# shubhamchandak94/HARC

Hardware: AMD Instinct MI355X
Metric: Mreads/s reorder+encode, 100 bp (higher is better)
Workload: dtype u64 (2-bit packed bases, XOR+popcount)

## Files before the change

harc_amd/csrc/api.cpp:

```cpp
#include "internal.h"
#include <stdarg.h>
#include <chrono>
#include <stdlib.h>

static thread_local char g_err[512] = "";
void harc_set_error(const char *fmt, ...)
{
    va_list ap; va_start(ap, fmt); vsnprintf(g_err, sizeof g_err, fmt, ap); va_end(ap);
}
extern "C" const char *harc_amd_last_error(void) { return g_err; }

static size_t pool_hand_back(harc_amd_ctx *c, size_t from, size_t asked)
{
    size_t given = 0;
    for (size_t i = 0; i < c->pool.size(); i++) {
        harc_amd_ctx::PoolChunk &k = c->pool[i];
        if (i == from || k.size == 0 || k.used != 0) continue;
        (void)hipFree(k.base); c->pool_total -= k.size; given += k.size; k.base = nullptr; k.size = 0;
    }
    if (given) {
        (void)hipGetLastError();
        if (getenv("HARC_AMD_TRACE")) fprintf(stderr, "[pool] %.2f GB of empty chunks handed back for a request of %.2f GB\n", given / 1e9, asked / 1e9);
    }
    return given;
// ... 166 lines not shown
}

extern "C" void harc_amd_destroy(harc_amd_ctx *c)
{
    if (!c) return;
    (void)hipSetDevice(c->P.device);
    if (c->stream) { (void)hipStreamSynchronize(c->stream); }
    if (c->copy_stream) { (void)hipStreamSynchronize(c->copy_stream); }
    delete c->comm; c->comm = nullptr;
    for (void *p : c->owned) (void)hipFree(p);
    for (auto &k : c->pool) (void)hipFree(k.base);
    for (auto &k : c->harena) (void)hipHostFree(k.base);
    if (c->feed_ring) (void)hipHostFree(c->feed_ring);
    if (c->stream) (void)hipStreamDestroy(c->stream);
    if (c->copy_stream) (void)hipStreamDestroy(c->copy_stream);
    if (c->ev_copy) (void)hipEventDestroy(c->ev_copy);
    delete c;
}

void harc_drop_results(harc_amd_ctx *c)
{
    harc_pool_release(c, 0);
    c->d_order = nullptr; c->d_flag = c->d_pos = c->d_rc = nullptr; c->d_order_s = nullptr; c->d_oreads = nullptr; c->d_sreads = nullptr;
    c->have_s1 = c->have_s2 = c->s1_from_files = false; c->M = c->S = 0;
    c->d_s2_order = c->d_s2_orderN = nullptr; c->n_s2_order = c->n_s2_orderN = 0;
    for (auto it = c->out.begin(); it != c->out.end();) { if (it->first.first < HARC_AMD_IN_ORDER_N) it = c->out.erase(it); else ++it; }
    harc_host_reset(c);
}

int harc_in_reserve(harc_amd_ctx *c, harc_amd_ctx::InBuf *b, size_t bytes)
{
    if (b->p && b->cap >= bytes) return HARC_AMD_OK;
    if (b->p) { harc_raw_free(c, b->p); b->p = nullptr; b->cap = 0; }
    RC_TRY(harc_raw_alloc(c, &b->p, bytes));
    b->cap = bytes;
    return HARC_AMD_OK;
}
void harc_reset_shard(harc_amd_ctx *c)
{
    c->d_reads = (uint64_t *)c->own_reads.p; c->N = c->N_own;
    c->d_nreads3 = (uint64_t *)c->own_nreads3.p; c->NN = c->NN_own;
    c->d_gid = c->d_ngid = nullptr;
    c->replicated = false;
    memset(c->shard_info, 0, sizeof c->shard_info);
    c->C.n_clean = c->N; c->C.n_N = c->NN;
}

// ... 73 lines not shown
    HIP_TRY(hipSetDevice(c->P.device));
    harc_drop_results(c);
    const int L = c->P.readlen;
    c->M = M; c->S = S;
    RC_TRY(dalloc(c, &c->d_order, (size_t)M + 1)); RC_TRY(dalloc(c, &c->d_flag, (size_t)M + 1)); RC_TRY(dalloc(c, &c->d_pos, (size_t)M + 1));
    RC_TRY(dalloc(c, &c->d_rc, (size_t)M + 1)); RC_TRY(dalloc(c, &c->d_order_s, (size_t)S + 1));
    RC_TRY(dalloc(c, &c->d_oreads, (size_t)M * c->W + 1)); RC_TRY(dalloc(c, &c->d_sreads, (size_t)S * c->W + 1));
    if (M) {
        HIP_TRY(hipMemcpyAsync(c->d_order, order, (size_t)M * 4, hipMemcpyHostToDevice, c->stream));
        HIP_TRY(hipMemcpyAsync(c->d_flag, flag, M, hipMemcpyHostToDevice, c->stream));
        HIP_TRY(hipMemcpyAsync(c->d_pos, pos, M, hipMemcpyHostToDevice, c->stream));
        HIP_TRY(hipMemcpyAsync(c->d_rc, rc, M, hipMemcpyHostToDevice, c->stream));
        char *d = nullptr; RC_TRY(upload(c, temp_dna, (size_t)(M - 1) * (L + 1) + L, &d));
        RC_TRY(s1_pack_ascii(c, d, M, (uint32_t)L + 1, c->d_oreads));
        HIP_TRY(hipStreamSynchronize(c->stream)); harc_raw_free(c, d);
    }
    if (S) {
        HIP_TRY(hipMemcpyAsync(c->d_order_s, order_s, (size_t)S * 4, hipMemcpyHostToDevice, c->stream));
        char *d = nullptr; RC_TRY(upload(c, temp_dna_s, (size_t)(S - 1) * (L + 1) + L, &d));
        RC_TRY(s1_pack_ascii(c, d, S, (uint32_t)L + 1, c->d_sreads));
        HIP_TRY(hipStreamSynchronize(c->stream)); harc_raw_free(c, d);
    }
    HIP_TRY(hipStreamSynchronize(c->stream));
    c->have_s1 = true; c->s1_from_files = true;
    c->C.n_main = M; c->C.n_singleton = S;
    return HARC_AMD_OK;
}

extern "C" int harc_amd_pack_reads_device(harc_amd_ctx *c, const char *d_ascii, uint32_t n, uint32_t stride, uint64_t *d_out)
{
    if (!c || (n && (!d_ascii || !d_out)) || stride < (uint32_t)c->P.readlen) return HARC_AMD_EINVAL;
    HIP_TRY(hipSetDevice(c->P.device));
    RC_TRY(s1_pack_ascii(c, d_ascii, n, stride, d_out));
    HIP_TRY(hipStreamSynchronize(c->stream));
    return HARC_AMD_OK;
}
extern "C" int harc_amd_partition_reads_device(harc_amd_ctx *c, const uint64_t *d_packed, uint32_t n, uint32_t nb, uint64_t *d_out, uint64_t *d_counts)
{
    if (!c || nb == 0 || nb > 4096 || !d_counts || (n && (!d_packed || !d_out))) return HARC_AMD_EINVAL;
    HIP_TRY(hipSetDevice(c->P.device));
    return s1_partition_reads(c, d_packed, n, nb, d_out, reinterpret_cast<unsigned long long *>(d_counts));
}
extern "C" int harc_amd_bucket_reads_device(harc_amd_ctx *c, const uint64_t *d_packed, uint32_t n, uint32_t nb, uint32_t *d_out)
{
    if (!c || nb == 0 || (n && (!d_packed || !d_out))) return HARC_AMD_EINVAL;
    HIP_TRY(hipSetDevice(c->P.device));
    RC_TRY(s1_bucket_reads(c, d_packed, n, nb, d_out));
// ... 18 lines not shown

extern "C" int harc_amd_encode(harc_amd_ctx *c)
{
    if (!c) return HARC_AMD_EINVAL;
    if (!c->have_s1) { harc_set_error("harc_amd_encode: no stage-I result (call harc_amd_reorder or harc_amd_set_stage1_streams)"); return HARC_AMD_ESTATE; }
    HIP_TRY(hipSetDevice(c->P.device));
    const double t0 = now_ms();
    c->s2_part = false; c->s2_e0 = 0; c->s2_e1 = 0;
    uint32_t oi0 = 0, oi1 = 0xFFFFFFFFu;
    int simr = 0, simw = 0;
#ifdef HARC_AMD_EXPERIMENTS
    if (const char *e = getenv("HARC_AMD_S2_SIM")) { if (sscanf(e, "%d/%d", &simr, &simw) != 2 || simw < 2 || simr < 0 || simr >= simw) simw = 0; }
#endif
    const int s2p = getenv("HARC_AMD_S2_PART") ? atoi(getenv("HARC_AMD_S2_PART")) : 1;
    const bool real_part = c->replicated && c->comm && (c->comm->world > 1 || s2p == 2) && s2p != 0;
    if ((real_part || simw) && !c->s1_from_files) {
        const uint32_t E = (uint32_t)c->P.num_thr, wd = real_part ? (uint32_t)c->comm->world : (uint32_t)simw, rk = real_part ? (uint32_t)c->comm->rank : (uint32_t)simr;
        c->s2_world = (int)wd; c->s2_rank = (int)rk;
        c->s2_part = true; c->s2_e0 = (int)((uint64_t)E * rk / wd); c->s2_e1 = (int)((uint64_t)E * (rk + 1) / wd);
        uint32_t q = 1u + (uint32_t)((c->M - 1u) / E); if (q == 0) q = 1;
        const uint64_t a0 = (uint64_t)c->s2_e0 * q, a1 = (uint64_t)c->s2_e1 * q;
        oi0 = (uint32_t)(a0 > c->M ? c->M : a0); oi1 = (uint32_t)((uint32_t)c->s2_e1 >= E || a1 > c->M ? c->M : a1);
    }
    if (!c->s1_from_files) RC_TRY(stage1_make_oriented(c, oi0, oi1));
    RC_TRY(stage2_run(c));
    c->C.encode_ms = now_ms() - t0;
    c->C.total_ms += c->C.encode_ms;
    c->C.device_bytes_peak = c->dev_peak;
    c->have_s2 = true;
    return HARC_AMD_OK;
}

extern "C" int harc_amd_pack_order(harc_amd_ctx *c)
{
    if (!c) return HARC_AMD_EINVAL;
    if (!c->have_s2) { harc_set_error("harc_amd_pack_order: encode first"); return HARC_AMD_ESTATE; }
    HIP_TRY(hipSetDevice(c->P.device));
    return pack_order_run(c);
}

extern "C" int harc_amd_get_stream(harc_amd_ctx *c, int32_t id, int32_t shard, const void **ptr, size_t *len)
{
    if (!c || !ptr || !len) return HARC_AMD_EINVAL;
    *ptr = nullptr; *len = 0;
    HIP_TRY(hipSetDevice(c->P.device));
    auto key = std::make_pair((int)id, (int)shard);
    auto it = c->out.find(key);
    if (it == c->out.end()) {
        if (id >= HARC_AMD_S1_ORDER && id <= HARC_AMD_S1_DNA_SINGLETON) {
            if (!c->have_s1 || shard != 0) { harc_set_error("stream %d not available", id); return HARC_AMD_ESTATE; }
            std::vector<uint8_t> &b = out_buf(c, id, shard);
            const int L = c->P.readlen;
            bool made_oriented = false;
            switch (id) {
            case HARC_AMD_S1_ORDER: RC_TRY(harc_d2h(c, b, c->d_order, (size_t)c->M * 4)); break;
            case HARC_AMD_S1_FLAG: RC_TRY(harc_d2h(c, b, c->d_flag, c->M)); break;
            case HARC_AMD_S1_POS: RC_TRY(harc_d2h(c, b, c->d_pos, c->M)); break;
            case HARC_AMD_S1_RC: RC_TRY(harc_d2h(c, b, c->d_rc, c->M)); break;
            case HARC_AMD_S1_ORDER_SINGLETON: RC_TRY(harc_d2h(c, b, c->d_order_s, (size_t)c->S * 4)); break;
            case HARC_AMD_S1_DNA: {
                if (!c->d_oreads) { RC_TRY(stage1_make_oriented(c)); made_oriented = true; }
                const harc_mark_t mk = harc_pool_mark(c);
                char *d = nullptr; RC_TRY(dalloc(c, &d, (size_t)c->M * (L + 1) + 1));
                RC_TRY(s1_unpack_to_ascii(c, c->d_oreads, c->M, d));
                RC_TRY(harc_d2h(c, b, d, (size_t)c->M * (L + 1)));
                HIP_TRY(hipStreamSynchronize(c->stream)); harc_pool_release(c, mk); (void)made_oriented;
                break; }
            case HARC_AMD_S1_DNA_SINGLETON: {
                const harc_mark_t mk = harc_pool_mark(c);
                uint64_t *sr = c->d_sreads; bool tmp = false;
                if (!sr) { RC_TRY(dalloc(c, &sr, (size_t)c->S * c->W + 1)); tmp = true; RC_TRY(s1_orient(c, c->d_reads, c->d_order_s, nullptr, c->S, sr)); }
                char *d = nullptr; RC_TRY(dalloc(c, &d, (size_t)c->S * (L + 1) + 1));
                RC_TRY(s1_unpack_to_ascii(c, sr, c->S, d));
                RC_TRY(harc_d2h(c, b, d, (size_t)c->S * (L + 1)));
                HIP_TRY(hipStreamSynchronize(c->stream)); harc_pool_release(c, mk); (void)tmp;
                break; }
            }
            HIP_TRY(hipStreamSynchronize(c->stream));
            it = c->out.find(key);
        } else if ((id == HARC_AMD_S2_ORDER || id == HARC_AMD_S2_ORDER_N_PE) && shard == 0 && c->have_s2 && c->d_s2_order) {
            const uint32_t *d = id == HARC_AMD_S2_ORDER ? c->d_s2_order : c->d_s2_orderN;
            const size_t n = id == HARC_AMD_S2_ORDER ? c->n_s2_order : c->n_s2_orderN;
            uint8_t *hp = nullptr;
            RC_TRY(harc_host_alloc(c, (void **)&hp, n));
// ... 43 lines not shown
```

harc_amd/csrc/devutil.h:

```cpp
#pragma once
#include "internal.h"

#define HARC_GRID_ROW 16777215u
static inline dim3 harc_grid256(uint64_t n)
{
    uint64_t b = (n + 255) / 256;
    if (b == 0) b = 1;
    if (b <= HARC_GRID_ROW) return dim3((unsigned)b);
    return dim3(HARC_GRID_ROW, (unsigned)((b + HARC_GRID_ROW - 1) / HARC_GRID_ROW));
}
static inline dim3 harc_fold256(uint64_t nblocks)
{
    if (nblocks == 0) nblocks = 1;
    if (nblocks <= HARC_GRID_ROW) return dim3((unsigned)nblocks);
    return dim3(HARC_GRID_ROW, (unsigned)((nblocks + HARC_GRID_ROW - 1) / HARC_GRID_ROW));
}
static inline dim3 wave_grid(uint32_t n) { if (n <= (1u << 25)) return dim3(n ? n : 1u); return dim3(1u << 25, (n + (1u << 25) - 1) >> 25); }
__device__ __forceinline__ uint64_t harc_bid() { return (uint64_t)blockIdx.y * gridDim.x + blockIdx.x; }
__device__ __forceinline__ uint64_t harc_gid() { return ((uint64_t)blockIdx.y * gridDim.x + blockIdx.x) * blockDim.x + threadIdx.x; }
__device__ __forceinline__ uint32_t harc_gid32()
{
    if (gridDim.y == 1) return blockIdx.x * blockDim.x + threadIdx.x;
    const uint64_t g = harc_gid(); return g > 0xFFFFFFFEull ? 0xFFFFFFFFu : (uint32_t)g;
}
// ... 98 lines not shown
{
    const int r = nb - 64 * w;
    return r >= 64 ? ~(uint64_t)0 : (r <= 0 ? 0 : (((uint64_t)1 << r) - 1));
}
__device__ __forceinline__ uint64_t rev2(uint64_t x)
{
    x = __brevll(x);
    return ((x & 0xAAAAAAAAAAAAAAAAULL) >> 1) | ((x & 0x5555555555555555ULL) << 1);
}
template <int W> __device__ __forceinline__ void rc_words(const uint64_t (&a)[W], int L, uint64_t (&o)[W])
{
    uint64_t r[W];
#pragma unroll
    for (int w = 0; w < W; w++) r[w] = rev2(a[W - 1 - w]);
    const int s = 64 * W - 2 * L;
    const int ws = s >> 6, bs = s & 63;
#pragma unroll
    for (int w = 0; w < W; w++) {
        uint64_t lo = sel0<W>(r, w + ws), hi = sel0<W>(r, w + ws + 1);
        uint64_t v = bs ? ((lo >> bs) | (hi << (64 - bs))) : lo;
        o[w] = (~v) & lowmask_word(2 * L, w);
    }
}
__device__ __forceinline__ uint64_t spread32(uint64_t a)
{
    a &= 0xFFFFFFFFULL;
    a = (a | (a << 16)) & 0x0000FFFF0000FFFFULL;
    a = (a | (a << 8)) & 0x00FF00FF00FF00FFULL;
    a = (a | (a << 4)) & 0x0F0F0F0F0F0F0F0FULL;
    a = (a | (a << 2)) & 0x3333333333333333ULL;
    a = (a | (a << 1)) & 0x5555555555555555ULL;
    return a;
}
__device__ __forceinline__ uint32_t wave_sum_u32(uint32_t v)
{
#pragma unroll
    for (int o = 32; o > 0; o >>= 1) v += __shfl_xor(v, o, 64);
    return v;
}
__device__ __forceinline__ uint64_t shfl_u64(uint64_t x, int src)
{
    const uint32_t lo = __shfl((uint32_t)x, src, 64), hi = __shfl((uint32_t)(x >> 32), src, 64);
    return (uint64_t)lo | ((uint64_t)hi << 32);
}
__device__ __forceinline__ uint64_t shfl_u64_any(uint64_t x, int xormask)
{
// ... 42 lines not shown
```

harc_amd/csrc/internal.h:

```cpp
#pragma once
#include <hip/hip_runtime.h>
#include <stdint.h>
#include <stdio.h>
#include <string.h>
#include <map>
#include <string>
#include <utility>
#include <vector>
#include "../../include/harc_amd.h"

#define HARC_NONE 0xFFFFFFFFu
#define HARC_MAXW 8
#define HARC_MAXW3 12
#define HARC_MAXK (1u << 20)
#define HARC_LOOK_CHUNKS 16
#ifndef HARC_NSUGG
#define HARC_NSUGG 8
#endif

void harc_set_error(const char *fmt, ...);

#define HIP_TRY(expr)                                                                                          \
    do {                                                                                                       \
        hipError_t _e = (expr);                                                                                \
// ... 64 lines not shown
    std::vector<void *> owned;
    std::map<void *, size_t> sizes;
    struct PoolChunk { char *base; size_t size, used; };
    std::vector<PoolChunk> pool;
    size_t pool_cur = 0, pool_total = 0;

    uint32_t N = 0;  uint64_t *d_reads = nullptr;
    uint32_t NN = 0; uint64_t *d_nreads3 = nullptr;
    struct InBuf { void *p = nullptr; size_t cap = 0; };
    InBuf own_reads, own_nreads3;
    uint32_t N_own = 0, NN_own = 0;
    uint64_t nrec_own = 0;
    struct HarcComm *comm = nullptr;
    InBuf x_reads, x_nreads3, x_gid, x_ngid;
    uint32_t *d_gid = nullptr, *d_ngid = nullptr;
    int s2_world = 1, s2_rank = 0;
    bool s2_part = false; int s2_e0 = 0, s2_e1 = 0;
    bool replicated = false;
    uint64_t shard_info[8] = { 0, 0, 0, 0, 0, 0, 0, 0 };
    bool have_s1 = false;
    uint32_t M = 0, S = 0;
    uint32_t *d_order = nullptr; uint8_t *d_flag = nullptr, *d_pos = nullptr, *d_rc = nullptr; uint32_t *d_order_s = nullptr;
    uint64_t *d_oreads = nullptr;
    uint64_t *d_sreads = nullptr;
    bool s1_from_files = false;
    bool have_s2 = false;
    uint32_t *d_s2_order = nullptr, *d_s2_orderN = nullptr; size_t n_s2_order = 0, n_s2_orderN = 0;

    struct OutBuf { const uint8_t *ptr = nullptr; size_t len = 0; std::vector<uint8_t> own; };
    std::map<std::pair<int, int>, OutBuf> out;
    struct HostChunk { char *base; size_t size, used; };
    std::vector<HostChunk> harena;
    harc_amd_counters C;
    uint64_t digest[4] = { 0, 0, 0, 0 }; bool have_digest = false;

    char *feed_ring = nullptr; size_t feed_ring_bytes = 0;

    void *d_tmp = nullptr; size_t tmp_bytes = 0;
};

struct HarcComm {
    int world = 1, rank = 0;
    virtual ~HarcComm() {}
    virtual int allgather_u64(harc_amd_ctx *c, const uint64_t *in, int n, uint64_t *out) = 0;
    virtual int alltoallv(harc_amd_ctx *c, int narr, const void *const *send, const size_t *const *soff, const size_t *const *sbytes,
                          void *const *recv, const size_t *const *roff, const size_t *const *rbytes) = 0;
// ... 90 lines not shown
```

harc_amd/csrc/stage2.hip:

```cpp
#include "devutil.h"
#include <time.h>
#include <algorithm>
#include <stdlib.h>

#define TUPLE_NONE 0xFFFFFFFFFFFFFFFFULL

struct S2Args {
    int L, W, W3, thresh_s, maxsearch;
    int ds[2], de[2], kbits[2];
    uint32_t M, S, T, q, nC;
    uint64_t total;
    const uint64_t *oreads;
    const uint8_t *flag, *pos, *rc;
    const uint32_t *order;
    const uint64_t *cand3;
    const uint32_t *cand_order;
    uint8_t *head;
    uint64_t *gstart;
    uint8_t *cons;
    const uint32_t *chead;
    const HashSlot *slots[2]; uint64_t cap[2]; const uint32_t *ids[2];
    unsigned long long *best;
    unsigned long long *bestbin[2];
    const uint32_t *bloom[2]; int bloom_shift[2];
    int bloom_lbits, bloom_nwin;
    uint64_t *cons2;
    const uint64_t *cand2, *candN;
    uint4 *events;
    unsigned int *nevents; uint32_t maxevents;
    int trace;
    uint64_t col0, col1; uint32_t tile_base;
    const uint64_t *evwin;
    unsigned long long *cbb[2]; uint32_t *cpos[2], *ccnt[2]; unsigned long long *tminbin[2]; int compact;
    int binmax_on;
    unsigned long long *binmax[2];
// ... 101 lines not shown
}

#define CSTRIP 16
#define CTHREADS 128
#define CTILE (CTHREADS * CSTRIP)
#ifndef CCHUNK
#define CCHUNK 256
#endif
#ifndef CL0
#define CL0 4
#endif
#define CPLANES 32
#ifndef CSHALLOW
#define CSHALLOW 12
#endif
__global__ void k_consensus_tiles(S2Args s, uint32_t ntiles, uint32_t *tlo, uint32_t *thi)
{
    const uint32_t t = harc_gid32();
    if (t >= ntiles) return;
    const uint64_t X0 = (uint64_t)(t + s.tile_base) * CTILE, X1 = X0 + CTILE < s.total ? X0 + CTILE : s.total;
    thi[t] = (uint32_t)ub_le(s.gstart, (long long)s.M, X1 - 1);
    tlo[t] = X0 >= (uint64_t)s.L ? (uint32_t)(ub_le(s.gstart, (long long)s.M, X0 - (uint64_t)s.L) + 1) : 0u;
}
template <int NPL> __device__ __forceinline__ bool consensus_tile(const S2Args &s, const uint32_t tile, const uint32_t *cid, const unsigned long long *cinfo, int want_windows, const uint32_t *tlo, const uint32_t *thi)
{
    extern __shared__ uint64_t cl_words[];
    int *const cl_g = reinterpret_cast<int *>(cl_words + (size_t)CCHUNK * s.W);
    const uint32_t *const cl_w32 = reinterpret_cast<const uint32_t *>(cl_words);
    const uint64_t X0 = (uint64_t)(tile + s.tile_base) * CTILE;
    const int L = s.L, W = s.W;
    const long long ilo = tlo[tile], ihi = thi[tile];
    const int x0r = (int)threadIdx.x * CSTRIP;
    const uint64_t x0 = X0 + (uint64_t)x0r;
    const bool mine = x0 < s.total;
    const int ncol = !mine ? 0 : x0 + CSTRIP <= s.total ? CSTRIP : (int)(s.total - x0);
    const int xlr = x0r + ncol - 1;
    const uint32_t EVEN = 0x55555555u;
    uint32_t lo[2][CL0], pl[2][NPL];
#pragma unroll
    for (int j = 0; j < CL0; j++) lo[0][j] = lo[1][j] = 0;
#pragma unroll
    for (int j = 0; j < NPL; j++) pl[0][j] = pl[1][j] = 0;
    bool ovf = false;
    int pend = 0, depth = CL0;
    auto flush = [&]() {
        uint32_t ca = 0, cb = 0;
#pragma unroll
        for (int j = 0; j < CL0; j++) {
            const uint32_t xa = pl[0][j] ^ lo[0][j], xb = pl[1][j] ^ lo[1][j];
            const uint32_t na = (pl[0][j] & lo[0][j]) | (xa & ca), nb = (pl[1][j] & lo[1][j]) | (xb & cb);
            pl[0][j] = xa ^ ca; pl[1][j] = xb ^ cb; ca = na; cb = nb;
            lo[0][j] = lo[1][j] = 0;
        }
// ... 6 lines not shown
            pl[0][j] ^= ca; pl[1][j] ^= cb; ca = ta; cb = tb;
            if (depth < j + 1) depth = j + 1;
        }
        if (NPL > CSHALLOW) {
#ifndef HARC_CONS_FIXED_DEPTH
            if (__builtin_amdgcn_ballot_w64((ca | cb) != 0) != 0)
#endif
            {
#pragma unroll
                for (int j = CSHALLOW; j < NPL; j++) {
                    const uint32_t ta = pl[0][j] & ca, tb = pl[1][j] & cb;
                    pl[0][j] ^= ca; pl[1][j] ^= cb; ca = ta; cb = tb;
                }
                depth = NPL;
            }
        } else ovf |= (ca | cb) != 0;
        pend = 0;
    };
    long long ilast = ilo - 1;
    int nstart = 0;
    for (long long base = ilo; base <= ihi; base += CCHUNK) {
        const int nch = (int)(ihi + 1 - base < CCHUNK ? ihi + 1 - base : CCHUNK);
        __syncthreads();
        for (int k = threadIdx.x; k < nch * W; k += CTHREADS) cl_words[k] = s.oreads[(size_t)base * W + k];
        for (int k = threadIdx.x; k < nch; k += CTHREADS) cl_g[k] = (int)((long long)s.gstart[base + k] - (long long)X0);
        __syncthreads();
        int k = nch;
        if (mine) {
            int a = -1, b = nch;
            while (b - a > 1) { const int mid = (a + b) >> 1; if (cl_g[mid] <= x0r - L) a = mid; else b = mid; }
            k = b;
        }
        auto start_of = [&](int kk) { return kk < nch ? cl_g[kk] : 0x7FFFFFFF; };
        auto window_of = [&](int kk, int g, uint32_t &w0, uint32_t &w1) {
            const int o0 = x0r - g, j0 = o0 < 0 ? 0 : o0;
            const uint32_t *r = cl_w32 + (size_t)(kk < nch ? kk : nch - 1) * (2 * W) + (j0 >> 4);
            w0 = r[0]; w1 = r[1];
        };
        int g = start_of(k), gn = start_of(k + 1);
        uint32_t w0, w1;
        window_of(k, g, w0, w1);
        for (;; k++) {
            const bool act = g <= xlr;
            if (__builtin_amdgcn_ballot_w64(act) == 0) break;
            uint32_t w0n, w1n;
            window_of(k + 1, gn, w0n, w1n);
            const int gnn = start_of(k + 2);
            if (act) {
// ... 53 lines not shown
                const uint64_t x = x0 + c;
                while (gnext <= x) { i++; gnext = i + 1 < (long long)s.M ? s.gstart[i + 1] : ~0ull; moved = true; }
                if (moved) {
                    const uint32_t k = cid[i] + (uint32_t)s.head[i] - 1u;
                    if (k != kprev) { ci = cinfo[k]; kprev = k; }
                    moved = false;
                }
                if (!(ci >> 63) && x + (uint64_t)L <= (ci & ~(1ULL << 63))) vmask |= 1u << c;
            }
        }
    }
#pragma unroll
    for (int c = 0; c < CSTRIP; c++) {
        if ((c & 3) == 0) outw[c >> 2] = 0;
        outw[c >> 2] |= (((indw >> (2 * c)) & 3u) | (((vmask >> c) & 1u) << 2)) << (8 * (c & 3));
    }
    if (ncol == CSTRIP) {
        *reinterpret_cast<uint4 *>(s.cons + x0) = make_uint4(outw[0], outw[1], outw[2], outw[3]);
    } else {
        for (int c = 0; c < ncol; c++) s.cons[x0 + c] = (uint8_t)(outw[c >> 2] >> (8 * (c & 3)));
    }
    return ovf;
}
template <int NPL> __global__ __launch_bounds__(CTHREADS, NPL == CPLANES ? 4 : 6) void k_consensus(S2Args s, const uint32_t *cid, const unsigned long long *cinfo, int want_windows, const uint32_t *tlo, const uint32_t *thi, uint32_t *tovf)
{
    if (NPL == CPLANES) {
        const uint32_t n = tovf[0];
        for (uint32_t k = blockIdx.x; k < n; k += gridDim.x) consensus_tile<NPL>(s, tovf[1 + k], cid, cinfo, want_windows, tlo, thi);
    } else {
        const bool ovf = consensus_tile<NPL>(s, blockIdx.x, cid, cinfo, want_windows, tlo, thi);
        if (__syncthreads_or(ovf) && threadIdx.x == 0) tovf[1 + atomicAdd(&tovf[0], 1u)] = blockIdx.x;
    }
}

__device__ __forceinline__ bool dict_lookup_b(const HashSlot *tab, uint64_t cap, uint64_t key, uint32_t *start, uint32_t *count)
{
    key = key_scramble(key);
    uint64_t sl = bucket_slot(key, cap);
    for (;;) {
        const uint4 r0 = *reinterpret_cast<const uint4 *>(&tab[sl]), r1 = *reinterpret_cast<const uint4 *>(&tab[sl + 1]);
        if (r0.w == 0) return false;
        if (((uint64_t)r0.x | ((uint64_t)r0.y << 32)) == key) { *start = r0.z; *count = r0.w; return true; }
        if (r1.w == 0) return false;
        if (((uint64_t)r1.x | ((uint64_t)r1.y << 32)) == key) { *start = r1.z; *count = r1.w; return true; }
        const uint4 r2 = *reinterpret_cast<const uint4 *>(&tab[sl + 2]), r3 = *reinterpret_cast<const uint4 *>(&tab[sl + 3]);
        if (r2.w == 0) return false;
        if (((uint64_t)r2.x | ((uint64_t)r2.y << 32)) == key) { *start = r2.z; *count = r2.w; return true; }
        if (r3.w == 0) return false;
        if (((uint64_t)r3.x | ((uint64_t)r3.y << 32)) == key) { *start = r3.z; *count = r3.w; return true; }
        if (!(r0.w & SLOT_OVF)) return false;
        sl += 4; if (sl >= cap) sl = 0;
    }
}
// ... 1132 lines not shown
int stage2_run(harc_amd_ctx *c)
{
    const harc_amd_params &P = c->P;
    const int L = P.readlen, W = c->W, W3 = c->W3;
    const uint32_t M = c->M, S = c->S, NN = c->NN, T = S + NN, E = (uint32_t)P.num_thr;
    for (auto it = c->out.begin(); it != c->out.end();) { if (it->first.first >= HARC_AMD_S2_SEQ) it = c->out.erase(it); else ++it; }
    const bool part = c->s2_part;
    HarcComm *const cm = (part && c->comm && c->replicated) ? c->comm : nullptr;
    const uint32_t pw = part ? (uint32_t)c->s2_world : 1u, pr = part ? (uint32_t)c->s2_rank : 0u;
    const uint32_t e0 = part ? (uint32_t)c->s2_e0 : 0u, e1 = part ? (uint32_t)c->s2_e1 : E;
    const uint32_t t0 = (uint32_t)((uint64_t)T * pr / pw), t1 = (uint32_t)((uint64_t)T * (pr + 1u) / pw);
    const bool trace2 = getenv("HARC_AMD_TRACE") != nullptr;
    struct timespec tl0; clock_gettime(CLOCK_MONOTONIC, &tl0);
    auto lap = [&](const char *what) { if (trace2) { (void)hipStreamSynchronize(c->stream); struct timespec t; clock_gettime(CLOCK_MONOTONIC, &t); fprintf(stderr, "[stage II%s] %s: %.1f ms\n", part ? " (partitioned)" : "", what, (t.tv_sec - tl0.tv_sec) * 1e3 + (t.tv_nsec - tl0.tv_nsec) * 1e-6); tl0 = t; } };

    S2Args a; memset(&a, 0, sizeof a);
    a.L = L; a.W = W; a.W3 = W3; a.thresh_s = P.thresh_s; a.maxsearch = P.maxsearch;
    if (L > 50) { a.ds[0] = 0; a.de[0] = 20; a.ds[1] = 21; a.de[1] = 41; }
    else { a.ds[0] = 0; a.de[0] = 20 * L / 50; a.ds[1] = 20 * L / 50 + 1; a.de[1] = 41 * L / 50; }
    for (int l = 0; l < 2; l++) a.kbits[l] = 3 * (a.de[l] - a.ds[l] + 1);
    a.M = M; a.S = S; a.T = T;
    a.q = 1u + (uint32_t)((M - 1u) / E);
    if (a.q == 0) a.q = 1;
    a.oreads = c->d_oreads; a.flag = c->d_flag; a.pos = c->d_pos; a.rc = c->d_rc; a.order = c->d_order;
    const uint32_t i0 = (uint32_t)((uint64_t)e0 * a.q > M ? M : (uint64_t)e0 * a.q), i1 = e1 >= E ? M : (uint32_t)((uint64_t)e1 * a.q > M ? M : (uint64_t)e1 * a.q);

    uint32_t *order_out = nullptr, *orderN_out = nullptr;
    RC_TRY(dalloc(c, &order_out, (size_t)(i1 - i0) + (size_t)S + 1)); RC_TRY(dalloc(c, &orderN_out, (size_t)NN + 1));
    c->d_s2_order = c->d_s2_orderN = nullptr; c->n_s2_order = c->n_s2_orderN = 0;
    PoolScope s2_scope(c);
    const bool want_digest = P.stream_digest != 0;
    unsigned long long *d_digest = nullptr;
    c->have_digest = false;
    if (want_digest) { RC_TRY(dalloc(c, &d_digest, 4)); HIP_TRY(hipMemsetAsync(d_digest, 0, 32, c->stream)); }

    uint64_t *cand3 = nullptr; uint32_t *cand_order = nullptr; unsigned long long *best = nullptr;
    RC_TRY(dalloc(c, &cand3, (size_t)T * W3 + 1)); RC_TRY(dalloc(c, &cand_order, (size_t)T + 1)); RC_TRY(dalloc(c, &best, (size_t)T + 1));
    if (S) {
        if (c->d_sreads) hipLaunchKernelGGL(k_cand3_from2, G256((size_t)S * W3), c->d_sreads, (const uint32_t *)nullptr, S, L, W, W3, cand3);
        else hipLaunchKernelGGL(k_cand3_from2, G256((size_t)S * W3), c->d_reads, c->d_order_s, S, L, W, W3, cand3);
    }
    if (NN) HIP_TRY(hipMemcpyAsync(cand3 + (size_t)S * W3, c->d_nreads3, (size_t)NN * W3 * 8, hipMemcpyDeviceToDevice, c->stream));
    if (T) hipLaunchKernelGGL(k_cand_order, G256(T), c->d_order_s, S, T, cand_order);
    HIP_TRY(hipMemsetAsync(best, 0xFF, ((size_t)T + 1) * 8, c->stream));
    a.cand3 = cand3; a.cand_order = cand_order; a.best = best;
    uint8_t *head = nullptr; uint32_t *u1 = nullptr; uint64_t *gstart = nullptr; uint32_t *chead = nullptr;
    RC_TRY(dalloc(c, &head, (size_t)M + 1)); RC_TRY(dalloc(c, &u1, (size_t)M + 1)); RC_TRY(dalloc(c, &gstart, (size_t)M + 1));
// ... 84 lines not shown
                HIP_TRY(hipMemcpyAsync(&hnd, nd, 8, hipMemcpyDeviceToHost, c->stream));
                HIP_TRY(hipStreamSynchronize(c->stream));
                if (hnd) { harc_set_error("stage II bitmap built by tiles differs from the one built with atomics in %llu words", hnd); return HARC_AMD_EINTERNAL; }
            }
        }
        HIP_TRY(hipStreamSynchronize(c->stream));
    }
    for (int l = 0; l < 2; l++) { a.slots[l] = dict[l].slots; a.cap[l] = dict[l].cap; a.ids[l] = dict[l].ids; a.bloom[l] = bloom[l]; a.bloom_shift[l] = bloom_shift[l]; }
    lap("candidates and their dictionaries (all candidates, on every rank)");

    uint8_t *h_seq = nullptr;
    struct CopyJoin { hipStream_t s; ~CopyJoin() { (void)hipStreamSynchronize(s); } } copy_join{ c->copy_stream };
    uint8_t *cons = nullptr; RC_TRY(dalloc(c, &cons, (size_t)total + 8));
    a.cons = cons;
    unsigned int nev = 0;
    if (col1 > col0) {
        unsigned long long *cinfo = nullptr; RC_TRY(dalloc(c, &cinfo, (size_t)nC + 1));
        hipLaunchKernelGGL(k_contig_info, G256(nC), a, cinfo);
        const uint32_t ntiles = (uint32_t)((col1 + CTILE - 1) / CTILE) - a.tile_base;
        uint32_t *tlo = nullptr, *thi = nullptr; RC_TRY(dalloc(c, &tlo, (size_t)ntiles + 1)); RC_TRY(dalloc(c, &thi, (size_t)ntiles + 1));
        hipLaunchKernelGGL(k_consensus_tiles, G256(ntiles), a, ntiles, tlo, thi);
        uint32_t *tovf = nullptr; RC_TRY(dalloc(c, &tovf, (size_t)ntiles + 1));
        HIP_TRY(hipMemsetAsync(tovf, 0, 4, c->stream));
        hipLaunchKernelGGL(k_consensus<CSHALLOW>, dim3(ntiles), dim3(CTHREADS), (size_t)CCHUNK * (W * 8 + 4), c->stream, a, (const uint32_t *)u1, (const unsigned long long *)cinfo, T ? 1 : 0,
                           (const uint32_t *)tlo, (const uint32_t *)thi, tovf);
        hipLaunchKernelGGL(k_consensus<CPLANES>, dim3(ntiles < 1024u ? ntiles : 1024u), dim3(CTHREADS), (size_t)CCHUNK * (W * 8 + 4), c->stream, a, (const uint32_t *)u1, (const unsigned long long *)cinfo, T ? 1 : 0,
                           (const uint32_t *)tlo, (const uint32_t *)thi, tovf);
        {
            const uint64_t soff = seq_total;
            uint64_t maxnb = 0;
            for (uint32_t e = e0; e < e1; e++) { seq_shards[e - e0] = SeqShard{ sh_col[e], seq_nb[e], seq_off[e] }; if (seq_nb[e] > maxnb) maxnb = seq_nb[e]; }
            if (maxnb) {
                SeqShard *d_shards = nullptr; RC_TRY(dalloc(c, &d_shards, (size_t)(e1 - e0)));
                HIP_TRY(hipMemcpyAsync(d_shards, seq_shards.data(), (size_t)(e1 - e0) * sizeof(SeqShard), hipMemcpyHostToDevice, c->stream));
                for (uint32_t y = 0; y < e1 - e0; y += 65535u)
                    hipLaunchKernelGGL(k_pack_seq, dim3((unsigned)((maxnb + 8 * 256 - 1) / (8 * 256)), e1 - e0 - y < 65535u ? e1 - e0 - y : 65535u), dim3(256), 0, c->stream, (const uint64_t *)cons2,
                                       (const SeqShard *)d_shards + y, seqpk);
            }
            for (uint32_t e = e0; e < e1; e++)
                if (seq_tl[e]) hipLaunchKernelGGL(k_bases_to_ascii, G256(seq_tl[e]), cons + sh_col[e] + 4 * seq_nb[e], seq_tl[e], seqpk + seq_off[e] + seq_nb[e]);
            HIP_TRY(hipGetLastError());
            if (want_digest) for (uint32_t e = e0; e < e1; e++) RC_TRY(digest_range(c, seqpk + seq_off[e], seq_nb[e] + seq_tl[e], 0x100 + e, d_digest + 0));
            RC_TRY(harc_host_alloc(c, (void **)&h_seq, (size_t)soff));
            HIP_TRY(hipEventRecord(c->ev_copy, c->stream));
            HIP_TRY(hipStreamWaitEvent(c->copy_stream, c->ev_copy, 0));
            if (soff) HIP_TRY(hipMemcpyAsync(h_seq, seqpk, (size_t)soff, hipMemcpyDeviceToHost, c->copy_stream));
        }
        if (T) {
            const dim3 rg(ntiles);
            auto propose = [&]() {
// ... 14 lines not shown
                RC_TRY(dalloc(c, &a.events, (size_t)a.maxevents));
                HIP_TRY(hipMemsetAsync(a.nevents, 0, 16, c->stream));
                propose();
                HIP_TRY(hipMemcpyAsync(&nev, a.nevents, 4, hipMemcpyDeviceToHost, c->stream));
                HIP_TRY(hipStreamSynchronize(c->stream));
                if (nev > a.maxevents) { harc_set_error("stage II: event count changed between two identical passes (%u > %u)", nev, a.maxevents); return HARC_AMD_EINTERNAL; }
            }
        }
    }
    HIP_TRY(hipGetLastError());
    unsigned long long *d_bdig = nullptr;
    auto best_digest = [&](const char *what) -> int {
        if (!getenv("HARC_AMD_TRACE") || !T) return HARC_AMD_OK;
        if (!d_bdig) RC_TRY(dalloc(c, &d_bdig, 2));
        unsigned long long hv = 0;
        HIP_TRY(hipMemsetAsync(d_bdig, 0, 8, c->stream));
        RC_TRY(digest_range(c, best, (uint64_t)T * 8, 0xBE57ull, d_bdig));
        HIP_TRY(hipMemcpyAsync(&hv, d_bdig, 8, hipMemcpyDeviceToHost, c->stream));
        HIP_TRY(hipStreamSynchronize(c->stream));
        fprintf(stderr, "[stage II] digest of the claims %s: %016llx (%u probes into large bins)\n", what, hv, nev);
        return HARC_AMD_OK;
    };
    RC_TRY(best_digest("after the proposals"));
    lap("consensus + read_seq + proposals (this rank's columns)");
    uint64_t *evwin = nullptr;
    if (nev) {
        RC_TRY(dalloc(c, &evwin, (size_t)nev * W3 + 1));
        WAVE_PER_ITEM(nev, hipLaunchKernelGGL(k_ev_windows, dim3(nb_), dim3(256), 0, c->stream, a, (const uint4 *)a.events, nev, evwin, kb_));
    }
    if (cm && T) {
        RC_TRY(cm->allreduce_min_u64(c, best, (size_t)T));
        RC_TRY(cm->wait(c, "all-reduce of the singleton / N-read claims"));
        std::vector<uint64_t> allnev((size_t)cm->world);
        { const uint64_t mine = nev; RC_TRY(cm->allgather_u64(c, &mine, 1, allnev.data())); }
        uint64_t tot = 0; for (uint64_t x : allnev) tot += x;
        if (tot > 0xFFFFFFFFull) { harc_set_error("stage II: more than 2^32 probes into large bins"); return HARC_AMD_EINVAL; }
        if (tot) {
            uint4 *ev_all = nullptr; uint64_t *win_all = nullptr;
            RC_TRY(dalloc(c, &ev_all, (size_t)tot + 1)); RC_TRY(dalloc(c, &win_all, (size_t)tot * W3 + 1));
            std::vector<size_t> so[2], sb[2], ro[2], rb[2];
            for (int k = 0; k < 2; k++) { so[k].assign(cm->world, 0); sb[k].resize(cm->world); ro[k].resize(cm->world); rb[k].resize(cm->world); }
            uint64_t acc = 0;
            for (int p = 0; p < cm->world; p++) {
                sb[0][p] = (size_t)nev * 16; sb[1][p] = (size_t)nev * W3 * 8;
                ro[0][p] = (size_t)acc * 16; rb[0][p] = (size_t)allnev[p] * 16; ro[1][p] = (size_t)acc * W3 * 8; rb[1][p] = (size_t)allnev[p] * W3 * 8;
                acc += allnev[p];
            }
// ... 338 lines not shown
```

Baseline: 778.0.

## Gather and orient reads inside consensus tiles instead of a separate oriented-copy pass

Stage II consensus tiles now fetch each read's packed words straight from the original read array through the order permutation. Reverse-complement is applied in shared memory, and the oriented words are written back for later use. This removes the separate stage1_make_oriented pass and its full read-and-write of the read set before encoding. In exchange, the tile loads become random gathers rather than contiguous copies, and the kernel is templated on the word count W. Another env switch can turn gathering off.

```diff
diff --git a/harc_amd/csrc/api.cpp b/harc_amd/csrc/api.cpp
--- a/harc_amd/csrc/api.cpp
+++ b/harc_amd/csrc/api.cpp
@@ -212,7 +212,7 @@
 {
     harc_pool_release(c, 0);
     c->d_order = nullptr; c->d_flag = c->d_pos = c->d_rc = nullptr; c->d_order_s = nullptr; c->d_oreads = nullptr; c->d_sreads = nullptr;
-    c->have_s1 = c->have_s2 = c->s1_from_files = false; c->M = c->S = 0;
+    c->have_s1 = c->have_s2 = c->s1_from_files = c->oreads_whole = c->s2_gather = false; c->M = c->S = 0;
     c->d_s2_order = c->d_s2_orderN = nullptr; c->n_s2_order = c->n_s2_orderN = 0;
     for (auto it = c->out.begin(); it != c->out.end();) { if (it->first.first < HARC_AMD_IN_ORDER_N) it = c->out.erase(it); else ++it; }
     harc_host_reset(c);
@@ -332,7 +332,7 @@
         HIP_TRY(hipStreamSynchronize(c->stream)); harc_raw_free(c, d);
     }
     HIP_TRY(hipStreamSynchronize(c->stream));
-    c->have_s1 = true; c->s1_from_files = true;
+    c->have_s1 = true; c->s1_from_files = true; c->oreads_whole = true;
     c->C.n_main = M; c->C.n_singleton = S;
     return HARC_AMD_OK;
 }
@@ -397,7 +397,17 @@
         const uint64_t a0 = (uint64_t)c->s2_e0 * q, a1 = (uint64_t)c->s2_e1 * q;
         oi0 = (uint32_t)(a0 > c->M ? c->M : a0); oi1 = (uint32_t)((uint32_t)c->s2_e1 >= E || a1 > c->M ? c->M : a1);
     }
-    if (!c->s1_from_files) RC_TRY(stage1_make_oriented(c, oi0, oi1));
+    const bool gather_on = getenv("HARC_AMD_S2_GATHER") ? atoi(getenv("HARC_AMD_S2_GATHER")) != 0 : true;
+    c->s2_gather = false;
+    if (!c->oreads_whole) {
+        if (gather_on) {
+            if (!c->d_oreads) RC_TRY(dalloc(c, &c->d_oreads, (size_t)c->M * c->W + 1));
+            c->s2_gather = true;
+        } else {
+            RC_TRY(stage1_make_oriented(c, oi0, oi1));
+            if (oi0 == 0 && oi1 >= c->M) c->oreads_whole = true;
+        }
+    }
     RC_TRY(stage2_run(c));
     c->C.encode_ms = now_ms() - t0;
     c->C.total_ms += c->C.encode_ms;
@@ -434,7 +444,7 @@
             case HARC_AMD_S1_RC: RC_TRY(harc_d2h(c, b, c->d_rc, c->M)); break;
             case HARC_AMD_S1_ORDER_SINGLETON: RC_TRY(harc_d2h(c, b, c->d_order_s, (size_t)c->S * 4)); break;
             case HARC_AMD_S1_DNA: {
-                if (!c->d_oreads) { RC_TRY(stage1_make_oriented(c)); made_oriented = true; }
+                if (!c->oreads_whole) { RC_TRY(stage1_make_oriented(c)); c->oreads_whole = true; made_oriented = true; }
                 const harc_mark_t mk = harc_pool_mark(c);
                 char *d = nullptr; RC_TRY(dalloc(c, &d, (size_t)c->M * (L + 1) + 1));
                 RC_TRY(s1_unpack_to_ascii(c, c->d_oreads, c->M, d));
diff --git a/harc_amd/csrc/devutil.h b/harc_amd/csrc/devutil.h
--- a/harc_amd/csrc/devutil.h
+++ b/harc_amd/csrc/devutil.h
@@ -144,6 +144,14 @@
         o[w] = (~v) & lowmask_word(2 * L, w);
     }
 }
+template <int W> __device__ __forceinline__ uint64_t rc_word_at(const uint64_t *a, int L, int w)
+{
+    const int s = 64 * W - 2 * L;
+    const int ws = s >> 6, bs = s & 63, j = w + ws;
+    const uint64_t lo = j < W ? rev2(a[W - 1 - j]) : 0, hi = j + 1 < W ? rev2(a[W - 2 - j]) : 0;
+    const uint64_t v = bs ? ((lo >> bs) | (hi << (64 - bs))) : lo;
+    return (~v) & lowmask_word(2 * L, w);
+}
 __device__ __forceinline__ uint64_t spread32(uint64_t a)
 {
     a &= 0xFFFFFFFFULL;
diff --git a/harc_amd/csrc/internal.h b/harc_amd/csrc/internal.h
--- a/harc_amd/csrc/internal.h
+++ b/harc_amd/csrc/internal.h
@@ -110,6 +110,8 @@
     uint32_t M = 0, S = 0;
     uint32_t *d_order = nullptr; uint8_t *d_flag = nullptr, *d_pos = nullptr, *d_rc = nullptr; uint32_t *d_order_s = nullptr;
     uint64_t *d_oreads = nullptr;
+    bool oreads_whole = false;
+    bool s2_gather = false;
     uint64_t *d_sreads = nullptr;
     bool s1_from_files = false;
     bool have_s2 = false;
diff --git a/harc_amd/csrc/stage2.hip b/harc_amd/csrc/stage2.hip
--- a/harc_amd/csrc/stage2.hip
+++ b/harc_amd/csrc/stage2.hip
@@ -11,6 +11,8 @@
     uint32_t M, S, T, q, nC;
     uint64_t total;
     const uint64_t *oreads;
+    const uint64_t *reads;
+    uint64_t *oreads_out;
     const uint8_t *flag, *pos, *rc;
     const uint32_t *order;
     const uint64_t *cand3;
@@ -158,13 +160,69 @@
     thi[t] = (uint32_t)ub_le(s.gstart, (long long)s.M, X1 - 1);
     tlo[t] = X0 >= (uint64_t)s.L ? (uint32_t)(ub_le(s.gstart, (long long)s.M, X0 - (uint64_t)s.L) + 1) : 0u;
 }
-template <int NPL> __device__ __forceinline__ bool consensus_tile(const S2Args &s, const uint32_t tile, const uint32_t *cid, const unsigned long long *cinfo, int want_windows, const uint32_t *tlo, const uint32_t *thi)
+#ifndef CGBATCH
+#define CGBATCH 4
+#endif
+template <int W, int B> __device__ __forceinline__ void consensus_gather(const S2Args &s, const long long base, const int nch, const uint64_t X0, uint64_t *cl_words, int *cl_g)
+{
+    constexpr int RPW = 64 / W, RPP = (CTHREADS / 64) * RPW;
+    constexpr int NPASS = (CCHUNK + RPP - 1) / RPP;
+    static_assert(NPASS <= 32 && CCHUNK <= 2 * CTHREADS, "a bit a pass in revmask; two starts a thread");
+    int tid = (int)threadIdx.x;
+    asm volatile("" : "+v"(tid));
+    const int lane = tid & 63, rl = lane / W, w = lane % W;
+    const int kk0 = (tid >> 6) * RPW + rl;
+    const bool lane_on = rl < RPW;
+    const int k0 = tid, k1 = k0 + CTHREADS;
+    unsigned long long g0 = 0, g1 = 0;
+    if (k0 < nch) g0 = s.gstart[base + k0];
+    if (k1 < nch) g1 = s.gstart[base + k1];
+    uint32_t revmask = 0;
+    for (int p0 = 0; p0 < NPASS && p0 * RPP < nch; p0 += B) {
+        uint32_t rid[B]; uint8_t rv[B]; uint64_t mine[B];
+#pragma unroll
+        for (int p = 0; p < B; p++) {
+            const int kk = kk0 + (p0 + p) * RPP;
+            rid[p] = 0; rv[p] = 0;
+            if (lane_on && kk < nch) { rid[p] = s.order[base + kk]; rv[p] = s.rc[base + kk]; }
+        }
+        if (p0 == 0) {
+            if (k0 < nch) cl_g[k0] = (int)((long long)g0 - (long long)X0);
+            if (k1 < nch) cl_g[k1] = (int)((long long)g1 - (long long)X0);
+        }
+#pragma unroll
+        for (int p = 0; p < B; p++) revmask |= (rv[p] == 'r' ? 1u : 0u) << (p0 + p);
+#pragma unroll
+        for (int p = 0; p < B; p++) {
+            const int kk = kk0 + (p0 + p) * RPP;
+            mine[p] = 0;
+            if (lane_on && kk < nch) mine[p] = s.reads[(size_t)rid[p] * W + w];
+        }
+#pragma unroll
+        for (int p = 0; p < B; p++) {
+            const int kk = kk0 + (p0 + p) * RPP;
+            if (lane_on && kk < nch) cl_words[kk * W + w] = mine[p];
+        }
+    }
+    __syncthreads();
+    for (int p = 0; p * RPP < nch; p++) {
+        const int kk = kk0 + p * RPP;
+        if (!(lane_on && kk < nch)) continue;
+        uint64_t ow = cl_words[kk * W + w];
+        if ((revmask >> p) & 1u) {
+            ow = rc_word_at<W>(cl_words + kk * W, s.L, w);
+            cl_words[kk * W + w] = ow;
+        }
+        if (cl_g[kk] >= 0) s.oreads_out[(size_t)(base + kk) * W + w] = ow;
+    }
+}
+template <int NPL, int GW> __device__ __forceinline__ bool consensus_tile(const S2Args &s, const uint32_t tile, const uint32_t *cid, const unsigned long long *cinfo, int want_windows, const uint32_t *tlo, const uint32_t *thi)
 {
     extern __shared__ uint64_t cl_words[];
-    int *const cl_g = reinterpret_cast<int *>(cl_words + (size_t)CCHUNK * s.W);
+    const int L = s.L, W = GW ? GW : s.W;
+    int *const cl_g = reinterpret_cast<int *>(cl_words + (size_t)CCHUNK * W);
     const uint32_t *const cl_w32 = reinterpret_cast<const uint32_t *>(cl_words);
     const uint64_t X0 = (uint64_t)(tile + s.tile_base) * CTILE;
-    const int L = s.L, W = s.W;
     const long long ilo = tlo[tile], ihi = thi[tile];
     const int x0r = (int)threadIdx.x * CSTRIP;
     const uint64_t x0 = X0 + (uint64_t)x0r;
@@ -217,8 +275,11 @@
     for (long long base = ilo; base <= ihi; base += CCHUNK) {
         const int nch = (int)(ihi + 1 - base < CCHUNK ? ihi + 1 - base : CCHUNK);
         __syncthreads();
-        for (int k = threadIdx.x; k < nch * W; k += CTHREADS) cl_words[k] = s.oreads[(size_t)base * W + k];
-        for (int k = threadIdx.x; k < nch; k += CTHREADS) cl_g[k] = (int)((long long)s.gstart[base + k] - (long long)X0);
+        if constexpr (GW != 0) consensus_gather<(GW ? GW : 1), (NPL == CPLANES || GW > 4 || GW == 3 ? 2 : CGBATCH)>(s, base, nch, X0, cl_words, cl_g);
+        else {
+            for (int k = threadIdx.x; k < nch * W; k += CTHREADS) cl_words[k] = s.oreads[(size_t)base * W + k];
+            for (int k = threadIdx.x; k < nch; k += CTHREADS) cl_g[k] = (int)((long long)s.gstart[base + k] - (long long)X0);
+        }
         __syncthreads();
         int k = nch;
         if (mine) {
@@ -318,13 +379,16 @@
     }
     return ovf;
 }
-template <int NPL> __global__ __launch_bounds__(CTHREADS, NPL == CPLANES ? 4 : 6) void k_consensus(S2Args s, const uint32_t *cid, const unsigned long long *cinfo, int want_windows, const uint32_t *tlo, const uint32_t *thi, uint32_t *tovf)
+#ifndef CGWAVES
+#define CGWAVES 6
+#endif
+template <int NPL, int GW> __global__ __launch_bounds__(CTHREADS, NPL == CPLANES ? 4 : GW ? CGWAVES : 6) void k_consensus(S2Args s, const uint32_t *cid, const unsigned long long *cinfo, int want_windows, const uint32_t *tlo, const uint32_t *thi, uint32_t *tovf)
 {
     if (NPL == CPLANES) {
         const uint32_t n = tovf[0];
-        for (uint32_t k = blockIdx.x; k < n; k += gridDim.x) consensus_tile<NPL>(s, tovf[1 + k], cid, cinfo, want_windows, tlo, thi);
+        for (uint32_t k = blockIdx.x; k < n; k += gridDim.x) consensus_tile<NPL, GW>(s, tovf[1 + k], cid, cinfo, want_windows, tlo, thi);
     } else {
-        const bool ovf = consensus_tile<NPL>(s, blockIdx.x, cid, cinfo, want_windows, tlo, thi);
+        const bool ovf = consensus_tile<NPL, GW>(s, blockIdx.x, cid, cinfo, want_windows, tlo, thi);
         if (__syncthreads_or(ovf) && threadIdx.x == 0) tovf[1 + atomicAdd(&tovf[0], 1u)] = blockIdx.x;
     }
 }
@@ -1503,7 +1567,7 @@
     a.M = M; a.S = S; a.T = T;
     a.q = 1u + (uint32_t)((M - 1u) / E);
     if (a.q == 0) a.q = 1;
-    a.oreads = c->d_oreads; a.flag = c->d_flag; a.pos = c->d_pos; a.rc = c->d_rc; a.order = c->d_order;
+    a.oreads = c->d_oreads; a.reads = c->s2_gather ? c->d_reads : nullptr; a.oreads_out = c->s2_gather ? c->d_oreads : nullptr; a.flag = c->d_flag; a.pos = c->d_pos; a.rc = c->d_rc; a.order = c->d_order;
     const uint32_t i0 = (uint32_t)((uint64_t)e0 * a.q > M ? M : (uint64_t)e0 * a.q), i1 = e1 >= E ? M : (uint32_t)((uint64_t)e1 * a.q > M ? M : (uint64_t)e1 * a.q);
 
     uint32_t *order_out = nullptr, *orderN_out = nullptr;
@@ -1634,10 +1698,18 @@
         hipLaunchKernelGGL(k_consensus_tiles, G256(ntiles), a, ntiles, tlo, thi);
         uint32_t *tovf = nullptr; RC_TRY(dalloc(c, &tovf, (size_t)ntiles + 1));
         HIP_TRY(hipMemsetAsync(tovf, 0, 4, c->stream));
-        hipLaunchKernelGGL(k_consensus<CSHALLOW>, dim3(ntiles), dim3(CTHREADS), (size_t)CCHUNK * (W * 8 + 4), c->stream, a, (const uint32_t *)u1, (const unsigned long long *)cinfo, T ? 1 : 0,
-                           (const uint32_t *)tlo, (const uint32_t *)thi, tovf);
-        hipLaunchKernelGGL(k_consensus<CPLANES>, dim3(ntiles < 1024u ? ntiles : 1024u), dim3(CTHREADS), (size_t)CCHUNK * (W * 8 + 4), c->stream, a, (const uint32_t *)u1, (const unsigned long long *)cinfo, T ? 1 : 0,
-                           (const uint32_t *)tlo, (const uint32_t *)thi, tovf);
+#define CONSENSUS_LAUNCH(GW) { \
+        hipLaunchKernelGGL((k_consensus<CSHALLOW, GW>), dim3(ntiles), dim3(CTHREADS), (size_t)CCHUNK * (W * 8 + 4), c->stream, a, (const uint32_t *)u1, (const unsigned long long *)cinfo, T ? 1 : 0, \
+                           (const uint32_t *)tlo, (const uint32_t *)thi, tovf); \
+        hipLaunchKernelGGL((k_consensus<CPLANES, GW>), dim3(ntiles < 1024u ? ntiles : 1024u), dim3(CTHREADS), (size_t)CCHUNK * (W * 8 + 4), c->stream, a, (const uint32_t *)u1, (const unsigned long long *)cinfo, T ? 1 : 0, \
+                           (const uint32_t *)tlo, (const uint32_t *)thi, tovf); }
+        if (!c->s2_gather) CONSENSUS_LAUNCH(0)
+        else switch (W) {
+            case 1: CONSENSUS_LAUNCH(1) break; case 2: CONSENSUS_LAUNCH(2) break; case 3: CONSENSUS_LAUNCH(3) break; case 4: CONSENSUS_LAUNCH(4) break;
+            case 5: CONSENSUS_LAUNCH(5) break; case 6: CONSENSUS_LAUNCH(6) break; case 7: CONSENSUS_LAUNCH(7) break; default: CONSENSUS_LAUNCH(8) break;
+        }
+#undef CONSENSUS_LAUNCH
+        if (c->s2_gather && !part) c->oreads_whole = true;
         {
             const uint64_t soff = seq_total;
             uint64_t maxnb = 0;
@@ -1698,7 +1770,7 @@
         return HARC_AMD_OK;
     };
     RC_TRY(best_digest("after the proposals"));
-    lap("consensus + read_seq + proposals (this rank's columns)");
+    lap(c->s2_gather ? "consensus (reads gathered by the tiles) + read_seq + proposals (this rank's columns)" : "consensus (reads staged from the oriented copy) + read_seq + proposals (this rank's columns)");
     uint64_t *evwin = nullptr;
     if (nev) {
         RC_TRY(dalloc(c, &evwin, (size_t)nev * W3 + 1));
```

Result: faster. 788.0 (median of 6 runs) (+1.3%).
